# INK-USC/RE-Net

Hardware: AMD Instinct MI355X
Metric: RGCN+GRU encoder triples/s at bs=1024 n_hidden=200 (full training step, both directions) (higher is better)
Workload: dtype f32; 1 GPU; ICEWS18-shaped synthetic stream (seed 999), n_hidden=200, seq_len=10, batch=1024 per GPU, dropout=0.50, fwd+bwd both directions + clip + Adam; parallelism=dp1, global_batch=1024, nodes=99312, edges=288792

## Files before the change

include/renet_hip.h:

```cpp
#ifndef RENET_HIP_H
#define RENET_HIP_H

#include <stddef.h>
#include <stdint.h>

#ifdef __cplusplus
extern "C" {
#endif

#define RENET_OK 0
#define RENET_ERR_BADARG (-1)
#define RENET_ERR_UNSUPPORTED (-2)
#define RENET_ERR_WORKSPACE (-3)

#define RENET_ABI_VERSION 1
int renet_version(void);

int renet_gather_rows(const float* table, const int32_t* idx, int n, int D, float* out, void* stream);
int renet_segment_add(const float* src, const int32_t* order, const int32_t* seg_ptr,
                      const int32_t* seg_target, int U, int D, float* dst, void* stream);
int renet_segment_add2(const float* src0, const float* src1, const int32_t* order, const int32_t* seg_ptr,
                       const int32_t* seg_target, int U, int D, float* dst0, float* dst1, void* stream);
#define RENET_SEGADD_MAX_JOBS 4
typedef struct {
    const int32_t *order, *seg_ptr, *seg_target;
    int U;
    float* dst;
    int dst_rows;
    int overwrite;
    const float *a0, *a1, *b;
} RenetSegAddJob;
int renet_segment_add_multi(int n, const RenetSegAddJob* jobs, int D, void* stream);

int renet_rgcn_gather(const float* x, int D, const int32_t* row_ptr, const int32_t* col,
                      const int32_t* etype, const float* scale, const float* W, int T, int type_shift,
                      int transpose_w, const float* addend, float drop_p, uint64_t seed, int relu,
                      float* out, int N, const int32_t* heavy_rows, int n_heavy, int heavy_thresh,
                      int src_limit, int addend_rows, void* stream);

int renet_rgcn_gather_items(const float* x, int D, const int32_t* it_src, const int32_t* it_type,
                            const int32_t* grp_ptr, int n_groups, const int32_t* row_ptr, const int32_t* col,
                            const int32_t* etype, const float* scale, const float* W, int T, int type_shift,
                            int transpose_w, const float* addend, float drop_p, uint64_t seed, int relu,
                            float* out, int N, const int32_t* heavy_rows, int n_heavy, int src_limit,
                            int addend_rows, int pruned, void* stream);

int renet_rgcn_gather_items_table(const float* table, int table_rows, int D, const int32_t* it_src_t,
                                  const int32_t* it_type_t, const int32_t* grp_ptr, int n_groups,
                                  const int32_t* row_ptr, const int32_t* col_t, const int32_t* etype,
                                  const int32_t* row_map, const float* scale, const float* W, int T, int type_shift,
                                  const float* addend_table, float drop_p, uint64_t seed, int relu, float* out, int N,
                                  const int32_t* heavy_rows, int n_heavy, void* stream);

int renet_rgcn_gather_items_bf16(const float* x, int D, const int32_t* it_src, const int32_t* it_type,
                                 const int32_t* grp_ptr, int n_groups, const int32_t* row_ptr, const int32_t* col,
// ... 67 lines not shown
int renet_gru_bwd_layouts_bf16out(int n, const float* const* dh_last, const int32_t* const* step_off, const int* L,
                                  int H, const float* const* Whh, const float* const* saved, void* const* dGi16,
                                  void* const* dGh16, int out_ld, float* workspace, size_t workspace_bytes,
                                  void* stream);
int renet_colsum_bf16(const void* X, int M, int N, int ldx, float* out, float beta, float* workspace,
                      size_t workspace_bytes, void* stream);
int renet_scale_bf16_by_device_scalar(void* x, size_t n, const float* scale, void* stream);

size_t renet_planes_elems(int R, int C);
int renet_pack_planes(const float* X, int R, int C, int ldx, int ones_col, void* out, void* stream);
int renet_gemm_planes(int a_tr, int b_tr, int M, int N, int K, float alpha, const float* alpha_dev, const void* Ap,
                      int lda, size_t a_plane, const void* Bp, int ldb, size_t b_plane, float beta, float* C, int ldc,
                      const float* bias, float* col_out, int split_k, float* workspace, size_t workspace_bytes,
                      void* stream);
int renet_softmax_ce_planes(const float* logits, const int32_t* target, int B, int C, int ld, float grad_scale,
                            float* row_loss, void* dl_planes, size_t plane, int ld16, int rows16, void* stream);
int renet_mix_ce_planes(const float* logits, const int32_t* target, const float* a_row, const float* q_row, int B, int C,
                        int ld, float grad_scale, float* row_loss, void* dl_planes, size_t plane, int ld16, int rows16,
                        float* d_a, void* stream);

size_t renet_colsum_workspace(int M, int N);
int renet_colsum(const float* X, int M, int N, int ldx, float* out, float beta, float* workspace,
                 size_t workspace_bytes, void* stream);

int renet_scale_by_device_scalar(float* x, size_t n, const float* scale, void* stream);
int renet_scale_by_device_scalar_bound(float* x, size_t n, const float* scale, float bound_in, float* bound_out,
                                       void* stream);

int renet_seq_assemble_fwd(const float* h2, const float* ent, const float* rel, const float* glob,
                           const int32_t* subj_row, const int32_t* row_ent, const int32_t* row_rel,
                           const int32_t* glob_row, int S, int D, float drop_p, uint64_t seed_x,
                           uint64_t seed_xr, float* X, float* Xr, void* stream);
int renet_bound_parts(size_t total4);
int renet_seq_assemble_fwd_bounds(const float* h2, const float* ent, const float* rel, const float* glob,
                                  const int32_t* subj_row, const int32_t* row_ent, const int32_t* row_rel,
                                  const int32_t* glob_row, int S, int D, float drop_p, uint64_t seed_x,
                                  uint64_t seed_xr, float* X, float* Xr, float* partX, float* partXr, void* stream);
int renet_seq_assemble_bwd(const float* dX, const float* dXr, const int32_t* step_off, int L, int S,
                           int B, int D, float drop_p, uint64_t seed_x, uint64_t seed_xr, float* dRows,
                           float* dEntSeq, float* dRelSeq, void* stream);

size_t renet_gru_workspace(int B, int H);
int renet_gru_fwd(const float* Gi, const int32_t* step_off, int L, int H, const float* Whh,
                  const float* bhh, float* h_last, int out_rows, float* saved, float* workspace,
                  size_t workspace_bytes, void* stream);
int renet_gru_bwd(const float* dh_last, const int32_t* step_off, int L, int H, const float* Whh,
// ... 327 lines not shown
```

re-net_amd/csrc/gemm.hip:

```cpp
#include <cstdint>
#include <cstdlib>
#include <type_traits>
#include "common.h"

namespace {

constexpr int BM = 128, BN = 128, BK = 32;
constexpr int LDK = BK + 4;
constexpr int LDR = BM + 4;
constexpr int OPBUF = BM * LDK;
constexpr int THREADS = 256;
static_assert(BK * LDR <= OPBUF, "operand buffer too small");

typedef float f32x16 __attribute__((ext_vector_type(16)));

struct GemmArgs {
    const float* A;
    const float* B;
    float* C;
    const float* bias;
    int M, N, K, lda, ldb, ldc;
    float alpha, beta;
    int k_tiles_per_split;
    int split_k;
// ... 510 lines not shown
inline int colsum_groups(int M) { return max(1, min(64, (M + 127) / 128)); }

template <typename T>
int colsum_impl(const T* X, int M, int N, int ldx, float* out, float beta, float* workspace,
                       size_t workspace_bytes, void* stream) {
    if (M < 0 || N <= 0 || ldx < N) return RENET_ERR_BADARG;
    const int G = colsum_groups(M);
    hipStream_t st = (hipStream_t)stream;
    if (G == 1) {
        RENET_LAUNCH((colsum_kernel<T>), dim3((N + 63) / 64, 1), dim3(256), 0, st, X, M, N, ldx, max(M, 1), beta, out);
        RENET_LAUNCH_CHECK();
        return RENET_OK;
    }
    if (workspace_bytes < (size_t)colsum_groups(M) * N * sizeof(float)) return RENET_ERR_WORKSPACE;
    const int rpg = (M + G - 1) / G;
    RENET_LAUNCH((colsum_kernel<T>), dim3((N + 63) / 64, G), dim3(256), 0, st, X, M, N, ldx, rpg, 0.f, workspace);
    RENET_LAUNCH_CHECK();
    RENET_LAUNCH((colsum_kernel<float>), dim3((N + 63) / 64, 1), dim3(256), 0, st, (const float*)workspace, G, N, N, G,
                 beta, out);
    RENET_LAUNCH_CHECK();
    return RENET_OK;
}


bool generic_forced() {
    static const bool v = renet_env_flag("RENET_GEMM_F32_GENERIC", false);
    return v;
}

}

extern "C" {

size_t renet_gemm_workspace(int M, int N, int split_k) {
    return split_k > 1 ? (size_t)split_k * (size_t)M * (size_t)N * sizeof(float) : 0;
}

int renet_gemm_f32(int ta, int tb, int M, int N, int K, float alpha, const float* A, int lda,
                   const float* B, int ldb, float beta, float* C, int ldc, const float* bias,
                   int split_k, float* workspace, size_t workspace_bytes, void* stream) {
    if (M < 0 || N < 0 || K < 0 || lda <= 0 || ldb <= 0 || ldc < N) return RENET_ERR_BADARG;
    if (M == 0 || N == 0) return RENET_OK;
    if (split_k < 1) split_k = 1;
    const int kt_total = (K + BK - 1) / BK;
    if (split_k > kt_total) split_k = max(kt_total, 1);
    if (split_k > 1 && workspace_bytes < renet_gemm_workspace(M, N, split_k)) return RENET_ERR_WORKSPACE;
// ... 51 lines not shown
int renet_scale_by_device_scalar(float* x, size_t n, const float* scale, void* stream) {
    if (!x || !scale || (reinterpret_cast<uintptr_t>(x) & 15)) return RENET_ERR_BADARG;
    if (n == 0) return RENET_OK;
    const int blocks = (int)min((size_t)2048, (n / 4 + 255) / 256 + 1);
    RENET_LAUNCH(scale_dev_kernel, dim3(blocks), dim3(256), 0, (hipStream_t)stream, x, n, scale, 0.f, (float*)nullptr);
    RENET_LAUNCH_CHECK();
    return RENET_OK;
}

int renet_scale_by_device_scalar_bound(float* x, size_t n, const float* scale, float bound_in, float* bound_out,
                                       void* stream) {
    if (!x || !scale || !bound_out || (reinterpret_cast<uintptr_t>(x) & 15)) return RENET_ERR_BADARG;
    const int blocks = (int)min((size_t)2048, (n / 4 + 255) / 256 + 1);
    RENET_LAUNCH(scale_dev_kernel, dim3(blocks), dim3(256), 0, (hipStream_t)stream, x, n, scale, bound_in, bound_out);
    RENET_LAUNCH_CHECK();
    return RENET_OK;
}

int renet_colsum(const float* X, int M, int N, int ldx, float* out, float beta, float* workspace,
                 size_t workspace_bytes, void* stream) {
    return colsum_impl<float>(X, M, N, ldx, out, beta, workspace, workspace_bytes, stream);
}

int renet_colsum_bf16(const void* X, int M, int N, int ldx, float* out, float beta, float* workspace,
                      size_t workspace_bytes, void* stream) {
    return colsum_impl<__bf16>((const __bf16*)X, M, N, ldx, out, beta, workspace, workspace_bytes, stream);
}

int renet_scale_bf16_by_device_scalar(void* x, size_t n, const float* scale, void* stream) {
    if (n == 0) return RENET_OK;
    const int blocks = (int)min((size_t)2048, (n + 255) / 256);
    RENET_LAUNCH(scale_dev_bf16_kernel, dim3(blocks), dim3(256), 0, (hipStream_t)stream, (__bf16*)x, n, scale);
    RENET_LAUNCH_CHECK();
    return RENET_OK;
}

}
```

re-net_amd/csrc/rows.hip:

```cpp
#include "common.h"

namespace {

__global__ __launch_bounds__(256) void gather_rows_kernel(const float4* __restrict__ table,
                                                          const int32_t* __restrict__ idx, int n, int CH,
                                                          float4* __restrict__ out) {
    const size_t total = (size_t)n * CH;
    for (size_t i = (size_t)blockIdx.x * blockDim.x + threadIdx.x; i < total;
         i += (size_t)gridDim.x * blockDim.x) {
        const int r = (int)(i / CH), c = (int)(i % CH);
        out[i] = table[(size_t)idx[r] * CH + c];
    }
}

constexpr int kSegWaves = 16, kSegShort = 16, kSegUnr = 8;
__global__ __launch_bounds__(kSegWaves * 64) void segment_add_kernel(const float4* __restrict__ src0,
                                                                     const float4* __restrict__ src1,
                                                                     const int32_t* __restrict__ order,
                                                                     const int32_t* __restrict__ seg_ptr,
                                                                     const int32_t* __restrict__ seg_target,
                                                                     int U, int CH, float4* __restrict__ dst0,
                                                                     float4* __restrict__ dst1) {
    const float4* __restrict__ src = blockIdx.y ? src1 : src0;
    float4* __restrict__ dst = blockIdx.y ? dst1 : dst0;
// ... 128 lines not shown
        const int k0 = J.seg_ptr[u], k1 = J.seg_ptr[u + 1];
        if (k1 - k0 <= kSegShort) continue;
        const size_t tgt = (size_t)__builtin_amdgcn_readfirstlane(J.seg_target[u]) * CH;
        for (int st = 0; st < stages; ++st) {
            const float4* s0 = st ? J.b : J.a0;
            const float4* s1 = st ? nullptr : J.a1;
            for (int ch = lane; ch < CH; ch += 64)
                red[wave][ch] = seg_stage_sum(s0, s1, J.order, CH, ch, k0 + wave * kSegUnr, k1, kSegWaves * kSegUnr);
            __syncthreads();
            if (wave == 0) {
                for (int ch = lane; ch < CH; ch += 64) {
                    float4 r = red[0][ch];
#pragma unroll 5
                    for (int w = 1; w < kSegWaves; ++w) r = f4_add(r, red[w][ch]);
                    const float4 d = (st == 0 && J.overwrite) ? zero : J.dst[tgt + ch];
                    J.dst[tgt + ch] = f4_add(d, r);
                }
            }
            __syncthreads();
        }
    }
}

}

extern "C" {

int renet_version(void) { return RENET_ABI_VERSION; }

int renet_gather_rows(const float* table, const int32_t* idx, int n, int D, float* out, void* stream) {
    if (n < 0 || D <= 0 || (D & 3)) return RENET_ERR_BADARG;
    if (n == 0) return RENET_OK;
    const int CH = D / 4;
    const size_t total = (size_t)n * CH;
    int blocks = (int)min((size_t)2048, (total + 255) / 256);
    RENET_LAUNCH(gather_rows_kernel, dim3(blocks), dim3(256), 0, (hipStream_t)stream,
                       (const float4*)table, idx, n, CH, (float4*)out);
    RENET_LAUNCH_CHECK();
    return RENET_OK;
}

static int seg_grid(int U) { return U <= 512 ? U : max(512, (U + kSegWaves - 1) / kSegWaves); }

int renet_segment_add(const float* src, const int32_t* order, const int32_t* seg_ptr,
                      const int32_t* seg_target, int U, int D, float* dst, void* stream) {
    if (U < 0 || D <= 0 || (D & 3)) return RENET_ERR_BADARG;
    if (U == 0) return RENET_OK;
    if (D > 512) return RENET_ERR_UNSUPPORTED;
    RENET_LAUNCH(segment_add_kernel, dim3(seg_grid(U)), dim3(kSegWaves * 64), 0,
                       (hipStream_t)stream, (const float4*)src, (const float4*)src, order, seg_ptr, seg_target, U, D / 4,
                       (float4*)dst, (float4*)dst);
    RENET_LAUNCH_CHECK();
    return RENET_OK;
}

int renet_segment_add2(const float* src0, const float* src1, const int32_t* order, const int32_t* seg_ptr,
                       const int32_t* seg_target, int U, int D, float* dst0, float* dst1, void* stream) {
    if (U < 0 || D <= 0 || (D & 3)) return RENET_ERR_BADARG;
    if (U == 0) return RENET_OK;
    if (D > 512) return RENET_ERR_UNSUPPORTED;
    RENET_LAUNCH(segment_add_kernel, dim3(seg_grid(U), 2), dim3(kSegWaves * 64), 0,
                       (hipStream_t)stream, (const float4*)src0, (const float4*)src1, order, seg_ptr, seg_target, U, D / 4,
                       (float4*)dst0, (float4*)dst1);
    RENET_LAUNCH_CHECK();
    return RENET_OK;
}

int renet_segment_add_multi(int n, const RenetSegAddJob* jobs, int D, void* stream) {
    if (n < 1 || n > RENET_SEGADD_MAX_JOBS || !jobs || D <= 0 || (D & 3)) return RENET_ERR_BADARG;
    for (int i = 0; i < n; ++i) {
        const RenetSegAddJob& q = jobs[i];
        if (q.U < 0 || !q.dst || !q.a0) return RENET_ERR_BADARG;
        if (q.U > 0 && (!q.order || !q.seg_ptr || !q.seg_target)) return RENET_ERR_BADARG;
        if (q.overwrite && q.U != q.dst_rows) return RENET_ERR_BADARG;
        for (int k = 0; k < i; ++k)
            if (jobs[k].dst == q.dst) return RENET_ERR_BADARG;
    }
    if (D > 512) return RENET_ERR_UNSUPPORTED;
    SegJobsK js{};
    int blocks = 0;
    for (int i = 0; i < n; ++i) {
        const RenetSegAddJob& q = jobs[i];
        if (q.U == 0) continue;
        SegJobK& k = js.j[js.n++];
        k = {(const float4*)q.a0, (const float4*)q.a1, (const float4*)q.b, q.order, q.seg_ptr, q.seg_target, (float4*)q.dst,
             q.U, seg_grid(q.U), blocks, q.overwrite ? 1 : 0};
        blocks += k.nwg;
    }
    if (js.n == 0) return RENET_OK;
    RENET_LAUNCH(segment_add_multi_kernel, dim3(blocks), dim3(kSegWaves * 64), 0, (hipStream_t)stream, js, D / 4);
    RENET_LAUNCH_CHECK();
    return RENET_OK;
}

}
```

re-net_amd/csrc/step.cpp:

```cpp
#include <hip/hip_runtime.h>
#include <algorithm>
#include <cstdint>
#include <cstdlib>
#include <vector>
#include "common.h"

namespace {

int auto_split_k(int m, int n, int k) {
    const long tiles = (long)((m + 127) / 128) * ((n + 127) / 128);
    const int ktiles = (k + 31) / 32;
    if (tiles >= 256 || ktiles < 8) return 1;
    const int smax = std::max(1, std::min(128, ktiles / 4));
    const double per_slice = (double)m * (double)n * 2.7e-6;
    int best = 1;
    double best_t = -1.0;
    for (int s = 1; s <= smax; ++s) {
        const long rounds = (tiles * s + 511) / 512;
        const double t = (double)rounds * ((double)ktiles / (double)s + 6.0) + (s > 1 ? per_slice * s : 0.0);
        if (best_t < 0.0 || t < best_t - 1e-9) { best = s; best_t = t; }
    }
    return best;
}

// ... 9 lines not shown
        const long rounds = (tiles * s + 255) / 256;
        const double t = (double)rounds * ((double)ktiles / (double)s + 6.0) + (s > 1 ? per_slice * s : 0.0);
        if (best_t < 0.0 || t < best_t - 1e-9) { best = s; best_t = t; }
    }
    return best;
}

inline size_t up(size_t x) { return (x + 255) & ~(size_t)255; }
inline size_t fbytes(size_t rows, size_t cols) { return up(rows * cols * sizeof(float)); }

struct Lay {
    size_t out1, out2, X, Xr, sv0, sv1, feat1, feat2, dl1, dl2, featp1;
    size_t ew, gi0, gi1, hs0, hs1, logits, featp;
    size_t dfeat1, dfeat2, da1, da2, dh1, dh2, dc1, dgi0, dgi1, dgh0, dgh1, dX, dXr, d_rows, d_ent_seq, d_rel_seq, d_h2, gn2,
        gl2, dhN, gn1, gl1, dh1N, gs;
    size_t gru_ws, gemm_ws_main, gemm_ws_side, bwdw_ws, colsum_ws;
    size_t gru_ws_bytes, gemm_ws_bytes, bwdw_ws_bytes, colsum_ws_bytes;
    size_t dl_plane, dl_ld, dl_rows, featp_plane, featp_ld, featp1_plane, featp1_ld, logits_ld;
    size_t total;
};

bool use_planes(const RenetStepModel& m) { return m.lin_w_planes != nullptr; }

enum { kBatchSegAdd = 2, kBatchSplit = 4, kBatchPack = 16 };
int step_batch() {
    static const int v = renet_env_int("RENET_STEP_BATCH", 22, 0, 31);
    return v;
}

Lay layout(const RenetStepModel& m, const RenetStepBatch& b) {
    Lay L{};
    size_t o = 0;
    auto take = [&](size_t bytes) { const size_t at = o; o += up(bytes); return at; };
    const size_t D = m.D, N = b.N, nA = b.nA, S = b.S, B = b.B, NE = m.num_ent, C2 = m.C2;
    const bool pl = use_planes(m);
    L.out1 = take(fbytes(N, D));
    L.out2 = take(fbytes(nA, D));
    L.X = take(fbytes(S, 4 * D));
    L.Xr = take(fbytes(S, 3 * D));
    L.sv0 = take(fbytes(S, 5 * D));
    L.sv1 = take(fbytes(S, 5 * D));
    L.feat1 = take(fbytes(B, 3 * D));
    L.feat2 = take(fbytes(B, 2 * D));
    L.dl2 = take(fbytes(B, C2));
    if (pl) {
        L.dl_rows = (B + 255) & ~(size_t)255;
        L.dl_ld = (NE + 255) & ~(size_t)255;
        L.dl_plane = L.dl_rows * L.dl_ld;
        L.dl1 = take(3 * L.dl_plane * 2);
// ... 41 lines not shown
    L.gru_ws_bytes = 2 * renet_gru_workspace(bmax, m.D);
    L.gru_ws = take(std::max<size_t>(L.gru_ws_bytes, 4));
    size_t need = 4;
    auto g_ = [&](int mm, int nn, int kk) { need = std::max(need, renet_gemm_workspace(mm, nn, auto_split_k(mm, nn, kk))); };
    const int Di = m.D, Si = b.S, Bi = b.B, NEi = m.num_ent, nAi = b.nA, C2i = m.C2;
    g_(NEi, Di, Di); g_(nAi, Di, Di); g_(Si, 3 * Di, 4 * Di); g_(Si, 3 * Di, 3 * Di); g_(Bi, NEi, 3 * Di); g_(Bi, C2i, 2 * Di);
    g_(Bi, 3 * Di, NEi); g_(NEi, 3 * Di, Bi); g_(Bi, 2 * Di, C2i); g_(C2i, 2 * Di, Bi);
    g_(3 * Di, 4 * Di, Si); g_(3 * Di, 3 * Di, Si); g_(3 * Di, Di, Si); g_(Si, 3 * Di, 3 * Di); g_(Si, 2 * Di, 3 * Di);
    g_(Di, Di, nAi); g_(Di, Di, NEi);
    if (pl) {
        need = std::max(need, renet_gemm_workspace(Bi, 3 * Di, auto_split_k_planes(Bi, 3 * Di, NEi)));
        need = std::max(need, renet_gemm_workspace(NEi, 3 * Di + 1, auto_split_k_planes(NEi, 3 * Di + 1, Bi)));
        need = std::max(need, renet_gemm_workspace(Bi, NEi, auto_split_k_planes(Bi, NEi, 3 * Di)));
    }
    L.gemm_ws_bytes = need;
    L.gemm_ws_main = take(need);
    L.gemm_ws_side = take(need);
    L.bwdw_ws_bytes = std::max<size_t>(renet_rgcn_bwd_w_workspace(std::max(b.n_chunks, b.n_chunks2), m.D), 4);
    L.bwdw_ws = take(L.bwdw_ws_bytes);
    size_t cs = 4;
    cs = std::max(cs, renet_colsum_workspace(Bi, NEi));
    cs = std::max(cs, renet_colsum_workspace(Bi, C2i));
    cs = std::max(cs, renet_colsum_workspace(Si, 3 * Di));
    L.colsum_ws_bytes = cs;
    L.colsum_ws = take(cs);
    L.total = o;
    return L;
}

bool args_ok(const RenetStepModel* m, const RenetStepBatch* b) {
    if (!m || !b) return false;
    if (!(m->D == 100 || m->D == 200 || m->D == 300 || m->D == 400) || m->num_ent < 1 || m->T < 2 || m->C2 < 1) return false;
    if (b->N < 1 || b->nA < 1 || b->nA > b->N || b->S < 1 || b->B < 1 || b->L < 1 || !b->step_off_host) return false;
    const size_t big = (size_t)std::max(b->N, m->num_ent) * m->D * 4;
    return big < ((size_t)1 << 31);
}

hipEvent_t step_event(int i) {
    thread_local std::vector<hipEvent_t> ev;
    while ((int)ev.size() <= i) {
        hipEvent_t e = nullptr;
        if (hipEventCreateWithFlags(&e, hipEventDisableTiming) != hipSuccess) return nullptr;
        ev.push_back(e);
    }
    return ev[i];
}
// ... 194 lines not shown
    }

    {
        const float* dhl[2] = {F(L.dh1), F(L.dh2)};
        const int32_t* so[2] = {b.step_off_host, b.step_off_host};
        const int ls[2] = {b.L, b.L};
        const float* sv[2] = {F(L.sv0), F(L.sv1)};
        float* dgi[2] = {F(L.dgi0), F(L.dgi1)};
        float* dgh[2] = {F(L.dgh0), F(L.dgh1)};
        CK((presplit ? renet_gru_bwd_layouts_presplit : renet_gru_bwd_layouts)(2, dhl, so, ls, D, whh2, sv, dgi, dgh, F(L.gru_ws),
                                                                               L.gru_ws_bytes, s.main));
    }
    auto gru_param_grads = [&]() -> int {
        const float* xs[2] = {F(L.X), F(L.Xr)};
        const int in[2] = {4 * D, 3 * D};
        const size_t dgi[2] = {L.dgi0, L.dgi1}, dgh[2] = {L.dgh0, L.dgh1}, sv[2] = {L.sv0, L.sv1};
        float* gwih[2] = {m.g_wih, m.g_wih_r};
        float* gwhh[2] = {m.g_whh, m.g_whh_r};
        float* gbih[2] = {m.g_bih, m.g_bih_r};
        float* gbhh[2] = {m.g_bhh, m.g_bhh_r};
        for (int k = 0; k < 2; ++k) {
            CK(gemm(s.side, wss, L.gemm_ws_bytes, 1, 0, 3 * D, in[k], S, F(dgi[k]), 3 * D, xs[k], in[k], 1.f, gwih[k], in[k], nullptr));
            CK(gemm(s.side, wss, L.gemm_ws_bytes, 1, 0, 3 * D, D, S, F(dgh[k]), 3 * D, F(sv[k]) + 4 * D, 5 * D, 1.f, gwhh[k], D, nullptr));
            CK(colsum(F(dgi[k]), S, 3 * D, gbih[k], s.side));
            CK(colsum(F(dgh[k]), S, 3 * D, gbhh[k], s.side));
        }
        return 0;
    };
    auto gru_done = [&]() -> int {
        if (!ev_gru_done) return 0;
        return (int)hipEventRecord((hipEvent_t)ev_gru_done, s.side);
    };
    {
        s.fork();
        int rc_ = gru_param_grads();
        if (!rc_) rc_ = gru_done();
        if (rc_) return rc_;
    }
    CK(gemm(s.main, wsm, L.gemm_ws_bytes, 0, 0, S, 3 * D, 3 * D, F(L.dgi0), 3 * D, m.wih, 4 * D, 0.f, F(L.dX), 4 * D, nullptr));
    CK(gemm(s.main, wsm, L.gemm_ws_bytes, 0, 0, S, 2 * D, 3 * D, F(L.dgi1), 3 * D, m.wih_r, 3 * D, 0.f, F(L.dXr), 3 * D, nullptr));

    CK(renet_seq_assemble_bwd(F(L.dX), F(L.dXr), b.step_off, b.L, S, B, D, p, r->seed_x, r->seed_xr, F(L.d_rows), F(L.d_ent_seq),
                              F(L.d_rel_seq), s.main));
    if (batch & kBatchSegAdd) {
        const bool cover = b.plan_subj_row.num_segments == nA;
        if (!cover) CK(renet_zero(F(L.d_h2), (size_t)nA * D, s.main));
        const RenetSegAddJob jobs[3] = {
            {b.plan_r.order, b.plan_r.seg_ptr, b.plan_r.target, b.plan_r.num_segments, m.g_rel, 0, 0, F(L.dc1), nullptr,
// ... 50 lines not shown
```

re-net_amd/renet_hip.py:

```python
import contextlib
import ctypes
import functools
import os
import threading
import weakref

import torch

_HERE = os.path.dirname(os.path.abspath(__file__))
LIB_PATH = os.environ.get('RENET_HIP_LIB', os.path.join(_HERE, 'csrc', 'librenet_hip.so'))

_lib = None

c_int = ctypes.c_int
c_float = ctypes.c_float
c_void_p = ctypes.c_void_p
c_size_t = ctypes.c_size_t
c_u64 = ctypes.c_uint64

_GEMM_ARGS = [c_int, c_int, c_int, c_int, c_int, c_float, c_void_p, c_int, c_void_p, c_int,
              c_float, c_void_p, c_int, c_void_p, c_int, c_void_p, c_size_t, c_void_p]
_RGCN_BWD_W_ARGS = [c_void_p, c_void_p, c_void_p, c_void_p, c_void_p, c_void_p, c_int,
                    c_void_p, c_int, c_int, c_int, c_void_p, c_float, c_void_p, c_size_t, c_void_p]
_GRU_FWD_LAYOUTS_ARGS = [c_int, c_void_p, c_void_p, c_void_p, c_int, c_void_p, c_void_p, c_void_p,
                         c_void_p, c_void_p, c_void_p, c_size_t, c_void_p]
_GRU_BWD_LAYOUTS_ARGS = [c_int, c_void_p, c_void_p, c_void_p, c_int, c_void_p, c_void_p, c_void_p,
                         c_void_p, c_void_p, c_size_t, c_void_p]

_SIGNATURES = {
    'renet_version': (c_int, []),
    'renet_gather_rows': (c_int, [c_void_p, c_void_p, c_int, c_int, c_void_p, c_void_p]),
    'renet_segment_add': (c_int, [c_void_p, c_void_p, c_void_p, c_void_p, c_int, c_int, c_void_p, c_void_p]),
    'renet_segment_add2': (c_int, [c_void_p, c_void_p, c_void_p, c_void_p, c_void_p, c_int, c_int, c_void_p, c_void_p,
                                   c_void_p]),
    'renet_segment_add_multi': (c_int, [c_int, c_void_p, c_int, c_void_p]),
    'renet_step_batch_mask': (c_int, []),
    'renet_gru_split_weights': (c_int, [c_int, c_void_p, c_int, c_int, c_void_p, c_size_t, c_void_p]),
    'renet_gru_fwd_layouts_presplit': (c_int, _GRU_FWD_LAYOUTS_ARGS),
    'renet_gru_bwd_layouts_presplit': (c_int, _GRU_BWD_LAYOUTS_ARGS),
    'renet_rgcn_gather': (c_int, [c_void_p, c_int, c_void_p, c_void_p, c_void_p, c_void_p, c_void_p, c_int,
                                  c_int, c_int, c_void_p, c_float, c_u64, c_int, c_void_p, c_int, c_void_p,
                                  c_int, c_int, c_int, c_int, c_void_p]),
    'renet_rgcn_gather_items': (c_int, [c_void_p, c_int, c_void_p, c_void_p, c_void_p, c_int, c_void_p, c_void_p,
                                        c_void_p, c_void_p, c_void_p, c_int, c_int, c_int, c_void_p, c_float, c_u64,
                                        c_int, c_void_p, c_int, c_void_p, c_int, c_int, c_int, c_int, c_void_p]),
    'renet_rgcn_gather_items_bf16': (c_int, [c_void_p, c_int, c_void_p, c_void_p, c_void_p, c_int, c_void_p, c_void_p,
                                             c_void_p, c_void_p, c_void_p, c_int, c_int, c_int, c_int, c_void_p,
                                             c_float, c_u64, c_int, c_void_p, c_int, c_void_p, c_int, c_int, c_int,
                                             c_int, c_void_p]),
    'renet_rgcn_gather_items_table_bf16': (c_int, [c_void_p, c_int, c_int, c_int, c_void_p, c_void_p, c_void_p, c_int,
                                                   c_void_p, c_void_p, c_void_p, c_void_p, c_void_p, c_void_p, c_int,
                                                   c_int, c_int, c_void_p, c_float, c_u64, c_int, c_void_p, c_int,
                                                   c_void_p, c_int, c_void_p]),
    'renet_rgcn_gather_items_table': (c_int, [c_void_p, c_int, c_int, c_void_p, c_void_p, c_void_p, c_int, c_void_p,
                                              c_void_p, c_void_p, c_void_p, c_void_p, c_void_p, c_int, c_int, c_void_p,
                                              c_float, c_u64, c_int, c_void_p, c_int, c_void_p, c_int, c_void_p]),
    'renet_compose_table_items': (c_int, [c_void_p, c_void_p, c_void_p, c_int, c_void_p, c_void_p, c_int, c_void_p,
                                          c_void_p, c_void_p, c_void_p, c_void_p]),
# ... 23 lines not shown
    'renet_seq_assemble_fwd_bf16': (c_int, [c_void_p, c_void_p, c_void_p, c_void_p, c_void_p, c_void_p, c_void_p,
                                            c_void_p, c_int, c_int, c_float, c_u64, c_u64, c_void_p, c_int, c_void_p,
                                            c_int, c_int, c_void_p]),
    'renet_softmax_ce_bf16': (c_int, [c_void_p, c_void_p, c_int, c_int, c_int, c_float, c_void_p, c_void_p, c_int, c_int,
                                      c_void_p]),
    'renet_gru_bwd_layouts_bf16out': (c_int, [c_int, c_void_p, c_void_p, c_void_p, c_int, c_void_p, c_void_p, c_void_p,
                                              c_void_p, c_int, c_void_p, c_size_t, c_void_p]),
    'renet_colsum_bf16': (c_int, [c_void_p, c_int, c_int, c_int, c_void_p, c_float, c_void_p, c_size_t, c_void_p]),
    'renet_scale_bf16_by_device_scalar': (c_int, [c_void_p, c_size_t, c_void_p, c_void_p]),
    'renet_planes_elems': (c_size_t, [c_int, c_int]),
    'renet_pack_planes': (c_int, [c_void_p, c_int, c_int, c_int, c_int, c_void_p, c_void_p]),
    'renet_gemm_planes': (c_int, [c_int, c_int, c_int, c_int, c_int, c_float, c_void_p, c_void_p, c_int, c_size_t,
                                  c_void_p, c_int, c_size_t, c_float, c_void_p, c_int, c_void_p, c_void_p, c_int,
                                  c_void_p, c_size_t, c_void_p]),
    'renet_softmax_ce_planes': (c_int, [c_void_p, c_void_p, c_int, c_int, c_int, c_float, c_void_p, c_void_p, c_size_t,
                                        c_int, c_int, c_void_p]),
    'renet_step_workspace': (c_size_t, [c_void_p, c_void_p]),
    'renet_step_forward': (c_int, [c_void_p, c_void_p, c_void_p, c_void_p, c_void_p]),
    'renet_step_backward': (c_int, [c_void_p, c_void_p, c_void_p, c_void_p, c_int, c_void_p, c_void_p, c_void_p]),
    'renet_add_inplace': (c_int, [c_void_p, c_void_p, c_size_t, c_void_p]),
    'renet_zero': (c_int, [c_void_p, c_size_t, c_void_p]),
    'renet_colsum_workspace': (c_size_t, [c_int, c_int]),
    'renet_colsum': (c_int, [c_void_p, c_int, c_int, c_int, c_void_p, c_float, c_void_p, c_size_t, c_void_p]),
    'renet_scale_by_device_scalar': (c_int, [c_void_p, c_size_t, c_void_p, c_void_p]),
    'renet_scale_by_device_scalar_bound': (c_int, [c_void_p, c_size_t, c_void_p, c_float, c_void_p, c_void_p]),
    'renet_seq_assemble_fwd': (c_int, [c_void_p, c_void_p, c_void_p, c_void_p, c_void_p, c_void_p, c_void_p,
                                       c_void_p, c_int, c_int, c_float, c_u64, c_u64, c_void_p, c_void_p,
                                       c_void_p]),
    'renet_seq_assemble_fwd_bounds': (c_int, [c_void_p, c_void_p, c_void_p, c_void_p, c_void_p, c_void_p, c_void_p,
                                              c_void_p, c_int, c_int, c_float, c_u64, c_u64, c_void_p, c_void_p,
                                              c_void_p, c_void_p, c_void_p]),
    'renet_seq_assemble_bwd': (c_int, [c_void_p, c_void_p, c_void_p, c_int, c_int, c_int, c_int, c_float,
                                       c_u64, c_u64, c_void_p, c_void_p, c_void_p, c_void_p]),
    'renet_gru_workspace': (c_size_t, [c_int, c_int]),
    'renet_gru_fwd': (c_int, [c_void_p, c_void_p, c_int, c_int, c_void_p, c_void_p, c_void_p, c_int, c_void_p,
                              c_void_p, c_size_t, c_void_p]),
    'renet_gru_bwd': (c_int, [c_void_p, c_void_p, c_int, c_int, c_void_p, c_void_p, c_void_p, c_void_p,
                              c_void_p, c_size_t, c_void_p]),
    'renet_gru_fwd_multi': (c_int, [c_int, c_void_p, c_void_p, c_int, c_int, c_void_p, c_void_p, c_void_p,
                                    c_int, c_void_p, c_void_p, c_size_t, c_void_p]),
    'renet_gru_bwd_multi': (c_int, [c_int, c_void_p, c_void_p, c_int, c_int, c_void_p, c_void_p, c_void_p,
                                    c_void_p, c_void_p, c_size_t, c_void_p]),
    'renet_gru_fwd_layouts': (c_int, _GRU_FWD_LAYOUTS_ARGS),
    'renet_gru_bwd_layouts': (c_int, _GRU_BWD_LAYOUTS_ARGS),
    'renet_gru_bound_parts': (c_int, [c_int]),
    'renet_gru_bwd_layouts_bounds': (c_int, [c_int, c_void_p, c_void_p, c_void_p, c_int, c_void_p, c_void_p, c_void_p,
# ... 935 lines not shown
        fn = lib().renet_gemm_f32_split if md == 'bf16x6' else lib().renet_gemm_bf16 if md == 'bf16' else \
            lib().renet_gemm_f32
        _check(fn(int(ta), int(tb), m, n, k, float(alpha), a.data_ptr(), _ld(a), b.data_ptr(),
                  _ld(b), float(beta), out.data_ptr(), _ld(out), _f32(bias), split_k, _f32(ws),
                  ws_bytes, _stream()), 'gemm_f32')
    _gemm_timed_end(t0, ta, tb, m, n, k, split_k)
    return out


def colsum(x, out=None, beta=0.0):
    fn, what, t = (lib().renet_colsum_bf16, 'colsum_bf16', x.p) if isinstance(x, BF16Mat) else \
        (lib().renet_colsum, 'colsum', x)
    m, n = x.shape
    if out is None:
        if beta != 0.0:
            raise RenetHipError('beta != 0 needs an output tensor')
        out = torch.empty(n, device=t.device, dtype=torch.float32)
    nbytes = lib().renet_colsum_workspace(m, n)
    ws = torch.empty(nbytes // 4, device=t.device, dtype=torch.float32) if nbytes else None
    _check(fn(t.data_ptr(), m, n, _ld(t), _f32(out), float(beta), _f32(ws), nbytes, _stream()), what)
    return out


def scale_by_device_scalar(x, g, bound_in=None):
    if bound_in is not None and not isinstance(x, BF16Mat):
        if not x.is_contiguous():
            raise RenetHipError('scale_by_device_scalar needs a contiguous tensor')
        out = torch.empty(1, device=x.device, dtype=torch.float32)
        _check(lib().renet_scale_by_device_scalar_bound(_f32(x), x.numel(), _f32(g), float(bound_in), out.data_ptr(),
                                                        _stream()), 'scale_by_device_scalar_bound')
        return out
    if isinstance(x, BF16Mat):
        _check(lib().renet_scale_bf16_by_device_scalar(x.p.data_ptr(), x.p.numel(), _f32(g), _stream()),
               'scale_bf16_by_device_scalar')
        return x
    if not x.is_contiguous():
        raise RenetHipError('scale_by_device_scalar needs a contiguous tensor')
    _check(lib().renet_scale_by_device_scalar(_f32(x), x.numel(), _f32(g), _stream()), 'scale_by_device_scalar')
    return x


def seq_assemble_fwd(h2, ent, rel, glob, subj_row, row_ent, row_rel, glob_row, drop_p, seed_x, seed_xr):
    s, d = subj_row.numel(), h2.shape[1]
    x = torch.empty(s, 4 * d, device=h2.device, dtype=torch.float32)
    xr = torch.empty(s, 3 * d, device=h2.device, dtype=torch.float32)
    args = (_f32(h2), _f32(ent), _f32(rel), _f32(glob), _i32(subj_row), _i32(row_ent), _i32(row_rel), _i32(glob_row), s, d,
# ... 687 lines not shown
```

Measured before the change: 406,500 triples/s.

## Batch GRU bias colsums into one multi-job kernel and add wave-grouped segment add

Adds a multi-job column-sum kernel that computes the GRU bias gradients for both directions in one launch. Because the input and hidden r/z bias gradients are identical, the dgi colsum is written to both bias buffers and only the n-gate slice of dgh is summed, so less data is read. Also adds a new segment-add kernel in which each wave handles several short segments at once, with a separate path for long segments, selected by default through RENET_SEG_WAVES. The batch mask default now enables the colsum batching, at the cost of more code paths and a new workspace sizing.

```diff
diff --git a/include/renet_hip.h b/include/renet_hip.h
--- a/include/renet_hip.h
+++ b/include/renet_hip.h
@@ -31,6 +31,7 @@
     const float *a0, *a1, *b;
 } RenetSegAddJob;
 int renet_segment_add_multi(int n, const RenetSegAddJob* jobs, int D, void* stream);
+int renet_segment_waves(void);
 
 int renet_rgcn_gather(const float* x, int D, const int32_t* row_ptr, const int32_t* col,
                       const int32_t* etype, const float* scale, const float* W, int T, int type_shift,
@@ -144,6 +145,18 @@
 size_t renet_colsum_workspace(int M, int N);
 int renet_colsum(const float* X, int M, int N, int ldx, float* out, float beta, float* workspace,
                  size_t workspace_bytes, void* stream);
+
+#define RENET_COLSUM_MAX_JOBS 8
+typedef struct {
+    const float* X;
+    int N, ldx;
+    float* out;
+    float* out2;
+    int out2_cols;
+} RenetColsumJob;
+size_t renet_colsum_multi_workspace(int M, int total_N);
+int renet_colsum_multi(int n, const RenetColsumJob* jobs, int M, float beta, float* workspace, size_t workspace_bytes,
+                       void* stream);
 
 int renet_scale_by_device_scalar(float* x, size_t n, const float* scale, void* stream);
 int renet_scale_by_device_scalar_bound(float* x, size_t n, const float* scale, float bound_in, float* bound_out,
diff --git a/re-net_amd/csrc/gemm.hip b/re-net_amd/csrc/gemm.hip
--- a/re-net_amd/csrc/gemm.hip
+++ b/re-net_amd/csrc/gemm.hip
@@ -556,6 +556,66 @@
     return RENET_OK;
 }
 
+
+struct ColJobK {
+    const float* X;
+    float *out, *out2;
+    int N, ldx, out2_cols, blk0;
+};
+struct ColJobsK { ColJobK j[RENET_COLSUM_MAX_JOBS]; int n; };
+
+__global__ __launch_bounds__(256) void colsum_multi_kernel(const ColJobsK js, int M, int rows_per_group, float beta,
+                                                           int final_pass) {
+    __shared__ float red[4][64];
+    int ji = 0;
+#pragma unroll
+    for (int i = 1; i < RENET_COLSUM_MAX_JOBS; ++i)
+        if (i < js.n && (int)blockIdx.x >= js.j[i].blk0) ji = i;
+    const ColJobK& J = js.j[ji];
+    const float* __restrict__ X = J.X;
+    const int N = J.N, ldx = J.ldx;
+    const int lane = threadIdx.x & 63, wave = threadIdx.x >> 6;
+    const int n = ((int)blockIdx.x - J.blk0) * 64 + lane;
+    const int g = blockIdx.y;
+    const int m0 = g * rows_per_group, m1 = min(M, m0 + rows_per_group);
+    float s0 = 0.f, s1 = 0.f, s2 = 0.f, s3 = 0.f;
+    if (n < N) {
+        int m = m0 + wave;
+        for (; m + 28 < m1; m += 32) {
+            float a[8];
+#pragma unroll
+            for (int q = 0; q < 8; ++q) a[q] = X[(size_t)(m + 4 * q) * ldx + n];
+            s0 += a[0]; s1 += a[1]; s2 += a[2]; s3 += a[3];
+            s0 += a[4]; s1 += a[5]; s2 += a[6]; s3 += a[7];
+        }
+        for (; m + 12 < m1; m += 16) {
+            s0 += X[(size_t)m * ldx + n];
+            s1 += X[(size_t)(m + 4) * ldx + n];
+            s2 += X[(size_t)(m + 8) * ldx + n];
+            s3 += X[(size_t)(m + 12) * ldx + n];
+        }
+        for (; m < m1; m += 4) s0 += X[(size_t)m * ldx + n];
+    }
+    red[wave][lane] = (s0 + s1) + (s2 + s3);
+    __syncthreads();
+    if (wave == 0 && n < N) {
+        const float r = (red[0][lane] + red[1][lane]) + (red[2][lane] + red[3][lane]);
+        if (!final_pass) {
+            J.out[(size_t)g * N + n] = r;
+        } else {
+            float* o = J.out + n;
+            float r1 = r;
+            if (beta != 0.f) r1 += beta * (*o);
+            *o = r1;
+            if (n < J.out2_cols) {
+                float* o2 = J.out2 + n;
+                float r2 = r;
+                if (beta != 0.f) r2 += beta * (*o2);
+                *o2 = r2;
+            }
+        }
+    }
+}
 
 bool generic_forced() {
     static const bool v = renet_env_flag("RENET_GEMM_F32_GENERIC", false);
@@ -653,6 +713,49 @@
     return colsum_impl<float>(X, M, N, ldx, out, beta, workspace, workspace_bytes, stream);
 }
 
+size_t renet_colsum_multi_workspace(int M, int total_N) {
+    const int G = colsum_groups(M);
+    return G > 1 && total_N > 0 ? (size_t)G * total_N * sizeof(float) : 0;
+}
+
+int renet_colsum_multi(int n, const RenetColsumJob* jobs, int M, float beta, float* workspace, size_t workspace_bytes,
+                       void* stream) {
+    if (n < 1 || n > RENET_COLSUM_MAX_JOBS || !jobs || M < 0) return RENET_ERR_BADARG;
+    int total = 0;
+    for (int i = 0; i < n; ++i) {
+        const RenetColsumJob& q = jobs[i];
+        if (!q.X || !q.out || q.N <= 0 || q.ldx < q.N) return RENET_ERR_BADARG;
+        if (q.out2 ? (q.out2_cols < 1 || q.out2_cols > q.N) : q.out2_cols != 0) return RENET_ERR_BADARG;
+        total += q.N;
+    }
+    const int G = colsum_groups(M);
+    if (G > 1 && (!workspace || workspace_bytes < renet_colsum_multi_workspace(M, total))) return RENET_ERR_WORKSPACE;
+    hipStream_t st = (hipStream_t)stream;
+    ColJobsK a{}, b{};
+    int blocks = 0;
+    size_t off = 0;
+    for (int i = 0; i < n; ++i) {
+        const RenetColsumJob& q = jobs[i];
+        float* slice = G > 1 ? workspace + off : nullptr;
+        a.j[i] = {q.X, G > 1 ? slice : q.out, G > 1 ? nullptr : q.out2, q.N, q.ldx, G > 1 ? 0 : q.out2_cols, blocks};
+        b.j[i] = {slice, q.out, q.out2, q.N, q.N, q.out2_cols, blocks};
+        blocks += (q.N + 63) / 64;
+        off += (size_t)G * q.N;
+    }
+    a.n = b.n = n;
+    if (G == 1) {
+        RENET_LAUNCH(colsum_multi_kernel, dim3(blocks, 1), dim3(256), 0, st, a, M, max(M, 1), beta, 1);
+        RENET_LAUNCH_CHECK();
+        return RENET_OK;
+    }
+    const int rpg = (M + G - 1) / G;
+    RENET_LAUNCH(colsum_multi_kernel, dim3(blocks, G), dim3(256), 0, st, a, M, rpg, 0.f, 0);
+    RENET_LAUNCH_CHECK();
+    RENET_LAUNCH(colsum_multi_kernel, dim3(blocks, 1), dim3(256), 0, st, b, G, G, beta, 1);
+    RENET_LAUNCH_CHECK();
+    return RENET_OK;
+}
+
 int renet_colsum_bf16(const void* X, int M, int N, int ldx, float* out, float beta, float* workspace,
                       size_t workspace_bytes, void* stream) {
     return colsum_impl<__bf16>((const __bf16*)X, M, N, ldx, out, beta, workspace, workspace_bytes, stream);
diff --git a/re-net_amd/csrc/rows.hip b/re-net_amd/csrc/rows.hip
--- a/re-net_amd/csrc/rows.hip
+++ b/re-net_amd/csrc/rows.hip
@@ -174,6 +174,159 @@
     }
 }
 
+
+enum { kSegAcc = 0, kSegOverwrite = 1 };
+
+__device__ __forceinline__ void seg_pin(float4& v) { asm volatile("" : "+v"(v.x), "+v"(v.y), "+v"(v.z), "+v"(v.w)); }
+
+__device__ __forceinline__ const float4* seg_at(const float4* row, int ch) {
+    return (const float4*)((const char*)row + (unsigned)ch * (unsigned)sizeof(float4));
+}
+__device__ __forceinline__ float4* seg_at(float4* row, int ch) {
+    return (float4*)((char*)row + (unsigned)ch * (unsigned)sizeof(float4));
+}
+
+template <int G, int R, bool TWO>
+__device__ __forceinline__ void seg_group_sum(const float4* __restrict__ a0, const float4* __restrict__ a1, int CH, int ch,
+                                              const int* ord, const int* len, int maxlen, float4* s) {
+#pragma unroll
+    for (int g = 0; g < G; ++g) s[g] = make_float4(0.f, 0.f, 0.f, 0.f);
+    for (int p = 0; p < maxlen; p += R) {
+        float4 v[G][R];
+        float4 w[G][R];
+#pragma unroll
+        for (int g = 0; g < G; ++g)
+#pragma unroll
+            for (int q = 0; q < R; ++q) {
+                const size_t at = (size_t)__builtin_amdgcn_readlane(ord[g], max(min(p + q, len[g] - 1), 0)) * CH;
+                v[g][q] = *seg_at(a0 + at, ch);
+                if (TWO) w[g][q] = *seg_at(a1 + at, ch);
+            }
+#pragma unroll
+        for (int g = 0; g < G; ++g)
+#pragma unroll
+            for (int q = 0; q < R; ++q) {
+                seg_pin(v[g][q]);
+                if (TWO) {
+                    seg_pin(w[g][q]);
+                    v[g][q] = f4_add(v[g][q], w[g][q]);
+                }
+            }
+#pragma unroll
+        for (int g = 0; g < G; ++g)
+#pragma unroll
+            for (int q = 0; q < R; ++q)
+                if (p + q < len[g]) s[g] = f4_add(s[g], v[g][q]);
+    }
+}
+
+#define SEG_ZERO4 make_float4(zs, zs, zs, zs)
+template <int G>
+__global__ __launch_bounds__(kSegWaves * 64, 8) void segment_waves_kernel(const SegJobsK js, int CH) {
+    constexpr int SL = kSegWaves * G;
+    __shared__ float4 red[kSegWaves][128];
+    __shared__ int s_k0[SL], s_k1[SL], s_tg[SL];
+    __shared__ unsigned long long s_long;
+    int ji = 0;
+#pragma unroll
+    for (int i = 1; i < RENET_SEGADD_MAX_JOBS; ++i)
+        if (i < js.n && (int)blockIdx.x >= js.j[i].blk0) ji = i;
+    const SegJobK& J = js.j[ji];
+    const int lane = threadIdx.x & 63;
+    const int wave = __builtin_amdgcn_readfirstlane(threadIdx.x >> 6);
+    const int bl = blockIdx.x - J.blk0, nwg = J.nwg, U = J.U, mode = J.overwrite;
+    float zs;
+    asm volatile("s_mov_b32 %0, 0" : "=s"(zs));
+    if (wave == 0) {
+        const int u = bl + lane * nwg;
+        const bool in = lane < SL && u < U;
+        const int uc = in ? u : 0;
+        const int k0 = J.seg_ptr[uc], k1 = J.seg_ptr[uc + 1], tg = J.seg_target[uc];
+        if (lane < SL) {
+            s_k0[lane] = in ? k0 : 0;
+            s_k1[lane] = in ? k1 : -1;
+            s_tg[lane] = in ? tg : 0;
+        }
+        const unsigned long long lm = __ballot(in && k1 - k0 > kSegShort);
+        if (lane == 0) s_long = lm;
+    }
+    __syncthreads();
+    {
+        int len[G], ord[G], tg[G];
+        int maxlen = 0;
+        bool any = false;
+#pragma unroll
+        for (int g = 0; g < G; ++g) {
+            const int sl = wave + kSegWaves * g;
+            const int n = __builtin_amdgcn_readfirstlane(s_k1[sl]) - __builtin_amdgcn_readfirstlane(s_k0[sl]);
+            tg[g] = __builtin_amdgcn_readfirstlane(s_tg[sl]);
+            len[g] = (n <= kSegShort && (n > 0 || (n == 0 && mode))) ? n : -1;
+            maxlen = max(maxlen, len[g]);
+            any |= len[g] >= 0;
+        }
+        if (any) {
+#pragma unroll
+            for (int g = 0; g < G; ++g) {
+                const int k0 = __builtin_amdgcn_readfirstlane(s_k0[wave + kSegWaves * g]);
+                ord[g] = maxlen > 0 ? J.order[max(k0 + min(lane, len[g] - 1), 0)] : 0;
+            }
+            constexpr int R = kSegUnr / G;
+            for (int ch = lane; ch < CH; ch += 64) {
+                float4 sa[G], d[G];
+                float4* drow[G];
+#pragma unroll
+                for (int g = 0; g < G; ++g) drow[g] = J.dst + (size_t)tg[g] * CH;
+                if (J.a1) seg_group_sum<G, R / 2, true>(J.a0, J.a1, CH, ch, ord, len, maxlen, sa);
+                else seg_group_sum<G, R, false>(J.a0, nullptr, CH, ch, ord, len, maxlen, sa);
+#pragma unroll
+                for (int g = 0; g < G; ++g) d[g] = *seg_at(drow[g], ch);
+#pragma unroll
+                for (int g = 0; g < G; ++g) d[g] = f4_add(mode ? SEG_ZERO4 : d[g], sa[g]);
+                if (J.b) {
+#pragma unroll
+                    for (int h = 0; h < G; h += 2) {
+                        seg_group_sum<2, 2, false>(J.b, nullptr, CH, ch, ord + h, len + h, maxlen, sa);
+#pragma unroll
+                        for (int g = 0; g < 2; ++g) d[h + g] = f4_add(d[h + g], sa[g]);
+                    }
+                }
+#pragma unroll
+                for (int g = 0; g < G; ++g)
+                    if (len[g] >= 0) *seg_at(drow[g], ch) = d[g];
+            }
+        }
+    }
+    const int stages = J.b ? 2 : 1;
+    unsigned long long lm = s_long;
+    lm = ((unsigned long long)(unsigned)__builtin_amdgcn_readfirstlane((int)(lm >> 32)) << 32) |
+         (unsigned)__builtin_amdgcn_readfirstlane((int)lm);
+    while (lm) {
+        const int j = __builtin_ctzll(lm);
+        lm &= lm - 1;
+        const int k0 = __builtin_amdgcn_readfirstlane(s_k0[j]), k1 = __builtin_amdgcn_readfirstlane(s_k1[j]);
+        const size_t tgt = (size_t)__builtin_amdgcn_readfirstlane(s_tg[j]) * CH;
+        for (int st = 0; st < stages; ++st) {
+            const float4* s0 = st ? J.b : J.a0;
+            const float4* s1 = st ? nullptr : J.a1;
+            for (int ch = lane; ch < CH; ch += 64)
+                red[wave][ch] = seg_stage_sum(s0, s1, J.order, CH, ch, k0 + wave * kSegUnr, k1, kSegWaves * kSegUnr);
+            __syncthreads();
+            if (wave == 0) {
+                for (int ch = lane; ch < CH; ch += 64) {
+                    float4 r = red[0][ch];
+#pragma unroll 5
+                    for (int w = 1; w < kSegWaves; ++w) r = f4_add(r, red[w][ch]);
+                    const float4 d = (st == 0 && mode) ? SEG_ZERO4 : J.dst[tgt + ch];
+                    J.dst[tgt + ch] = f4_add(d, r);
+                }
+            }
+            __syncthreads();
+        }
+    }
+}
+
+#undef SEG_ZERO4
+
 }
 
 extern "C" {
@@ -194,11 +347,38 @@
 
 static int seg_grid(int U) { return U <= 512 ? U : max(512, (U + kSegWaves - 1) / kSegWaves); }
 
+static int seg_waves() {
+    static const int v = renet_env_int("RENET_SEG_WAVES", 2, 0, 4);
+    return v == 0 ? 0 : v <= 2 ? 2 : 4;
+}
+static int seg_grid_waves(int U, int G) { return U <= 512 ? U : max(256, (U + kSegWaves * G - 1) / (kSegWaves * G)); }
+
+static int launch_seg_waves(SegJobsK& js, int G, int CH, hipStream_t st) {
+    int blocks = 0;
+    for (int i = 0; i < js.n; ++i) {
+        js.j[i].nwg = seg_grid_waves(js.j[i].U, G);
+        js.j[i].blk0 = blocks;
+        blocks += js.j[i].nwg;
+    }
+    if (G == 2) RENET_LAUNCH(segment_waves_kernel<2>, dim3(blocks), dim3(kSegWaves * 64), 0, st, js, CH);
+    else RENET_LAUNCH(segment_waves_kernel<4>, dim3(blocks), dim3(kSegWaves * 64), 0, st, js, CH);
+    RENET_LAUNCH_CHECK();
+    return RENET_OK;
+}
+
+int renet_segment_waves(void) { return seg_waves(); }
+
 int renet_segment_add(const float* src, const int32_t* order, const int32_t* seg_ptr,
                       const int32_t* seg_target, int U, int D, float* dst, void* stream) {
     if (U < 0 || D <= 0 || (D & 3)) return RENET_ERR_BADARG;
     if (U == 0) return RENET_OK;
     if (D > 512) return RENET_ERR_UNSUPPORTED;
+    if (const int G = seg_waves()) {
+        SegJobsK js{};
+        js.n = 1;
+        js.j[0] = {(const float4*)src, nullptr, nullptr, order, seg_ptr, seg_target, (float4*)dst, U, 0, 0, kSegAcc};
+        return launch_seg_waves(js, G, D / 4, (hipStream_t)stream);
+    }
     RENET_LAUNCH(segment_add_kernel, dim3(seg_grid(U)), dim3(kSegWaves * 64), 0,
                        (hipStream_t)stream, (const float4*)src, (const float4*)src, order, seg_ptr, seg_target, U, D / 4,
                        (float4*)dst, (float4*)dst);
@@ -211,6 +391,13 @@
     if (U < 0 || D <= 0 || (D & 3)) return RENET_ERR_BADARG;
     if (U == 0) return RENET_OK;
     if (D > 512) return RENET_ERR_UNSUPPORTED;
+    if (const int G = seg_waves()) {
+        SegJobsK js{};
+        js.n = 2;
+        js.j[0] = {(const float4*)src0, nullptr, nullptr, order, seg_ptr, seg_target, (float4*)dst0, U, 0, 0, kSegAcc};
+        js.j[1] = {(const float4*)src1, nullptr, nullptr, order, seg_ptr, seg_target, (float4*)dst1, U, 0, 0, kSegAcc};
+        return launch_seg_waves(js, G, D / 4, (hipStream_t)stream);
+    }
     RENET_LAUNCH(segment_add_kernel, dim3(seg_grid(U), 2), dim3(kSegWaves * 64), 0,
                        (hipStream_t)stream, (const float4*)src0, (const float4*)src1, order, seg_ptr, seg_target, U, D / 4,
                        (float4*)dst0, (float4*)dst1);
@@ -236,10 +423,11 @@
         if (q.U == 0) continue;
         SegJobK& k = js.j[js.n++];
         k = {(const float4*)q.a0, (const float4*)q.a1, (const float4*)q.b, q.order, q.seg_ptr, q.seg_target, (float4*)q.dst,
-             q.U, seg_grid(q.U), blocks, q.overwrite ? 1 : 0};
+             q.U, seg_grid(q.U), blocks, q.overwrite ? kSegOverwrite : kSegAcc};
         blocks += k.nwg;
     }
     if (js.n == 0) return RENET_OK;
+    if (const int G = seg_waves()) return launch_seg_waves(js, G, D / 4, (hipStream_t)stream);
     RENET_LAUNCH(segment_add_multi_kernel, dim3(blocks), dim3(kSegWaves * 64), 0, (hipStream_t)stream, js, D / 4);
     RENET_LAUNCH_CHECK();
     return RENET_OK;
diff --git a/re-net_amd/csrc/step.cpp b/re-net_amd/csrc/step.cpp
--- a/re-net_amd/csrc/step.cpp
+++ b/re-net_amd/csrc/step.cpp
@@ -55,9 +55,9 @@
 
 bool use_planes(const RenetStepModel& m) { return m.lin_w_planes != nullptr; }
 
-enum { kBatchSegAdd = 2, kBatchSplit = 4, kBatchPack = 16 };
+enum { kBatchColsum = 1, kBatchSegAdd = 2, kBatchSplit = 4, kBatchPack = 16 };
 int step_batch() {
-    static const int v = renet_env_int("RENET_STEP_BATCH", 22, 0, 31);
+    static const int v = renet_env_int("RENET_STEP_BATCH", 23, 0, 31);
     return v;
 }
 
@@ -145,6 +145,7 @@
     cs = std::max(cs, renet_colsum_workspace(Bi, NEi));
     cs = std::max(cs, renet_colsum_workspace(Bi, C2i));
     cs = std::max(cs, renet_colsum_workspace(Si, 3 * Di));
+    cs = std::max(cs, renet_colsum_multi_workspace(Si, 8 * Di));
     L.colsum_ws_bytes = cs;
     L.colsum_ws = take(cs);
     L.total = o;
@@ -385,8 +386,19 @@
         for (int k = 0; k < 2; ++k) {
             CK(gemm(s.side, wss, L.gemm_ws_bytes, 1, 0, 3 * D, in[k], S, F(dgi[k]), 3 * D, xs[k], in[k], 1.f, gwih[k], in[k], nullptr));
             CK(gemm(s.side, wss, L.gemm_ws_bytes, 1, 0, 3 * D, D, S, F(dgh[k]), 3 * D, F(sv[k]) + 4 * D, 5 * D, 1.f, gwhh[k], D, nullptr));
-            CK(colsum(F(dgi[k]), S, 3 * D, gbih[k], s.side));
-            CK(colsum(F(dgh[k]), S, 3 * D, gbhh[k], s.side));
+            if (!(batch & kBatchColsum)) {
+                CK(colsum(F(dgi[k]), S, 3 * D, gbih[k], s.side));
+                CK(colsum(F(dgh[k]), S, 3 * D, gbhh[k], s.side));
+            }
+        }
+        if (batch & kBatchColsum) {
+            RenetColsumJob jobs[4];
+            for (int k = 0; k < 2; ++k) {
+                jobs[2 * k] = {F(dgi[k]), 3 * D, 3 * D, gbih[k], gbhh[k], 2 * D};
+                jobs[2 * k + 1] = {F(dgh[k]) + 2 * D, D, 3 * D, gbhh[k] + 2 * D, nullptr, 0};
+            }
+            const size_t need = renet_colsum_multi_workspace(S, 8 * D);
+            CK(renet_colsum_multi(4, jobs, S, 1.f, need ? csw : nullptr, need, s.side));
         }
         return 0;
     };
diff --git a/re-net_amd/renet_hip.py b/re-net_amd/renet_hip.py
--- a/re-net_amd/renet_hip.py
+++ b/re-net_amd/renet_hip.py
@@ -34,6 +34,7 @@
     'renet_segment_add2': (c_int, [c_void_p, c_void_p, c_void_p, c_void_p, c_void_p, c_int, c_int, c_void_p, c_void_p,
                                    c_void_p]),
     'renet_segment_add_multi': (c_int, [c_int, c_void_p, c_int, c_void_p]),
+    'renet_segment_waves': (c_int, []),
     'renet_step_batch_mask': (c_int, []),
     'renet_gru_split_weights': (c_int, [c_int, c_void_p, c_int, c_int, c_void_p, c_size_t, c_void_p]),
     'renet_gru_fwd_layouts_presplit': (c_int, _GRU_FWD_LAYOUTS_ARGS),
@@ -103,6 +104,8 @@
     'renet_zero': (c_int, [c_void_p, c_size_t, c_void_p]),
     'renet_colsum_workspace': (c_size_t, [c_int, c_int]),
     'renet_colsum': (c_int, [c_void_p, c_int, c_int, c_int, c_void_p, c_float, c_void_p, c_size_t, c_void_p]),
+    'renet_colsum_multi_workspace': (c_size_t, [c_int, c_int]),
+    'renet_colsum_multi': (c_int, [c_int, c_void_p, c_int, c_float, c_void_p, c_size_t, c_void_p]),
     'renet_scale_by_device_scalar': (c_int, [c_void_p, c_size_t, c_void_p, c_void_p]),
     'renet_scale_by_device_scalar_bound': (c_int, [c_void_p, c_size_t, c_void_p, c_float, c_void_p, c_void_p]),
     'renet_seq_assemble_fwd': (c_int, [c_void_p, c_void_p, c_void_p, c_void_p, c_void_p, c_void_p, c_void_p,
@@ -1084,6 +1087,23 @@
     return out
 
 
+class ColsumJobC(ctypes.Structure):
+    _fields_ = [('X', c_void_p), ('N', c_int), ('ldx', c_int), ('out', c_void_p), ('out2', c_void_p), ('out2_cols', c_int)]
+
+
+def colsum_multi(jobs, beta=1.0):
+    arr = (ColsumJobC * max(len(jobs), 1))()
+    m, total, dev = 0, 0, None
+    for j, (x, out, out2, out2_cols) in zip(arr, jobs):
+        m, dev = x.shape[0], x.device
+        j.X, j.N, j.ldx = x.data_ptr(), x.shape[1], _ld(x)
+        j.out, j.out2, j.out2_cols = _f32(out), _f32(out2), int(out2_cols)
+        total += x.shape[1]
+    nbytes = lib().renet_colsum_multi_workspace(m, total)
+    ws = torch.empty(nbytes // 4, device=dev, dtype=torch.float32) if nbytes else None
+    return lib().renet_colsum_multi(len(jobs), ctypes.addressof(arr), m, float(beta), _f32(ws), nbytes, _stream())
+
+
 def scale_by_device_scalar(x, g, bound_in=None):
     if bound_in is not None and not isinstance(x, BF16Mat):
         if not x.is_contiguous():
```

New measurement: 405,200 triples/s. No clear change (-0.3%).
